# mcan1999/vulkan-raytracing

Measured on AMD Instinct MI355X. Metric: Mrays/sec (primary+secondary) at 1920×1080 depth 4; 1/2/4/8-GPU scaling, higher is better.
Workload: dtype f32

## Files before the change

### vulkan_raytracing_amd/csrc/kernels.hip

```cpp
#include <hip/hip_runtime.h>

#include "rt_kernels.h"
#include "../../include/rt_api.h"

namespace rt {

struct F3 { float x, y, z; };
__device__ __forceinline__ F3 mk3(float x, float y, float z) { F3 r; r.x = x; r.y = y; r.z = z; return r; }
__device__ __forceinline__ F3 add3(F3 a, F3 b) { return mk3(a.x + b.x, a.y + b.y, a.z + b.z); }
__device__ __forceinline__ F3 sub3(F3 a, F3 b) { return mk3(a.x - b.x, a.y - b.y, a.z - b.z); }
__device__ __forceinline__ F3 mul3(F3 a, float s) { return mk3(a.x * s, a.y * s, a.z * s); }
__device__ __forceinline__ F3 neg3(F3 a) { return mk3(-a.x, -a.y, -a.z); }
__device__ __forceinline__ float dot3(F3 a, F3 b) { return __builtin_fmaf(a.z, b.z, __builtin_fmaf(a.y, b.y, a.x * b.x)); }
__device__ __forceinline__ F3 cross3(F3 a, F3 b) {
  return mk3(__builtin_fmaf(a.y, b.z, -(a.z * b.y)), __builtin_fmaf(a.z, b.x, -(a.x * b.z)), __builtin_fmaf(a.x, b.y, -(a.y * b.x)));
}
__device__ __forceinline__ float length3(F3 v) { return __builtin_sqrtf(dot3(v, v)); }
__device__ __forceinline__ F3 normalize3(F3 v) { float inv = 1.0f / length3(v); return mul3(v, inv); }
__device__ __forceinline__ F3 fma3(float s, F3 a, F3 b) { return mk3(__builtin_fmaf(s, a.x, b.x), __builtin_fmaf(s, a.y, b.y), __builtin_fmaf(s, a.z, b.z)); }
__device__ __forceinline__ F3 reflect3(F3 I, F3 N) { float k = 2.0f * dot3(N, I); return fma3(-k, N, I); }

__device__ __forceinline__ F3 xform_point(const float* m, F3 p) {
  return mk3(__builtin_fmaf(m[2], p.z, __builtin_fmaf(m[1], p.y, m[0] * p.x)) + m[3],
             __builtin_fmaf(m[6], p.z, __builtin_fmaf(m[5], p.y, m[4] * p.x)) + m[7],
// ... 1159 lines not shown
    };
#else
    auto fast_step = [&]() {
      if (cur >= 0) {
        const uint4* np = reinterpret_cast<const uint4*>(node_bytes + ((uint32_t)cur << 5));
        const uint4 Q0 = np[0], Q1 = np[1];
        const int top = stk_lds[(sp - 1) * 64];
        const int2 ch = make_int2((int)Q1.z, (int)Q1.w);
        if (COUNT) cnt_nodes++;
        float t0, t1;
        const bool h0 = slab_q(Q0.x, Q0.y, Q0.z, qs, qb, rot, (RAYS8 ? tmin_ray : a.tmin), best_t, t0);
        const bool h1 = slab_q(Q0.w, Q1.x, Q1.y, qs, qb, rot, (RAYS8 ? tmin_ray : a.tmin), best_t, t1);
        const bool both = h0 && h1, none = !(h0 || h1), swap = t1 < t0;
        const uint32_t pm = 0u - (uint32_t)both;
        stk_lds[(((uint32_t)sp & pm) | ((uint32_t)STACK2_LDS & ~pm)) * 64u] = swap ? ch.x : ch.y;
        const int one = h0 ? ch.x : ch.y;
        cur = both ? (swap ? ch.y : ch.x) : (none ? top : one);
        sp += (both ? 1 : 0) - (none ? 1 : 0);
      }
    };
#endif
    constexpr int UNROLL = WIDE ? RT_WIDE_UNROLL : RT_INTERIOR_UNROLL;
    for (;;) {
      const uint32_t n_int = (uint32_t)__builtin_popcountll(__ballot(cur >= 0));
      if (n_int == 0 || n_int < keep_going) break;
#if !defined(RT_EXP_PHASE_SEL) && !defined(RT_EXP_VISIT_STAMPS)
      if (COUNT && lane == 0) { diag_iters++; diag_busy += n_int; }
#endif
      const bool deep = cur >= 0 && (sp + UNROLL > STACK2_LDS || far);
      if (!WIDE && __ballot(deep) == 0) {
#pragma unroll
        for (int r = 0; r < UNROLL; r++) fast_step();
      } else {
#pragma unroll
        for (int r = 0; r < UNROLL; r++) interior_step();
      }
    }

    PH_BEGIN(1)
    if (cur < 0 && cur > REF_MARK && cur_inst >= 0) {
      const bool any_ray = ANY || (QF && (qword & QF_TERMINATE) != 0u);
      for (int chain = 0; chain < RT_LEAF_CHAIN; chain++) {
        const uint32_t ref = (uint32_t)(~cur);
        const uint32_t first = ref >> 3, count = (ref & 7u) + 1u;
        for (uint32_t k = 0; k < count; k++) {
          const float4* tp = a.sc.tris + (size_t)(first + k) * 3;
          const float4 T0 = tp[0], T1 = tp[1], T2 = tp[2];
          if (COUNT) cnt_tris++;
          float tt, uu, vv;
          bool acc;
          if constexpr (QF) acc = tri_test_facing(T0, T1, T2, co, cd, tmin_ray, any_ray ? best_t : tmax, qword, tt, uu, vv);
          else acc = tri_test(T0, T1, T2, co, cd, (RAYS8 ? tmin_ray : a.tmin), (ANY ? best_t : ((ENTRY && MODE == MODE_CLOSEST) ? 10000.0f : tmax)), tt, uu, vv);
          if (acc) {
            if (ANY && MODE == MODE_SHADOW) best_inst = cur_inst;
            else {
              const int prim = (int)__float_as_uint(T2.y);
              const bool better = (best_inst < 0) || (tt < best_t) ||
                                  (tt == best_t && (cur_inst < best_inst || (cur_inst == best_inst && prim < best_prim)));
              if (better) { best_t = tt; best_u = uu; best_v = vv; best_prim = prim; best_inst = cur_inst; }
            }
          }
        }
        if (any_ray && best_inst >= 0) { cur = REF_DONE; break; }
        pop();
        if (!(cur < 0 && cur > REF_MARK)) break;
      }
    }
    PH_END(1)
    PH_BEGIN(2)
    if (cur == REF_MARK) {
      cur_inst = -1;
      pop();
      if (cur >= 0) { quant_space(wo, wd, a.sc.tlas_q_lo, a.sc.tlas_q_scale, qs, qb, rot); far = FAR && quant_far_o(wo, a.sc.tlas_q_lo, a.sc.tlas_q_scale); }
    }
    PH_END(2)
    PH_BEGIN(3)
    if (cur < 0 && cur > REF_MARK && cur_inst < 0) {
      const int ii = ~cur;
      int root; uint32_t imask;
      to_instance(ii, root, imask);
      bool skip = (imask & 0xFFu) == 0u;
      if (QF) {
        uint32_t cull;
        skip = !query_enters(qword, imask, cull);
        qword = (qword & ~(QF_CULL_NEG | QF_CULL_POS)) | cull;
      }
      if (skip) {
        pop();
        if (cur >= 0) { quant_space(wo, wd, a.sc.tlas_q_lo, a.sc.tlas_q_scale, qs, qb, rot); far = FAR && quant_far_o(wo, a.sc.tlas_q_lo, a.sc.tlas_q_scale); }
      } else {
        push(REF_MARK);
        cur_inst = ii; cur = root;
      }
    }

    PH_END(3)
    PH_BEGIN(4)
    const bool fin = !need && cur == REF_DONE;
    const uint64_t fin_mask = __ballot(fin);
    if (fin_mask != 0) {
      const uint32_t n_fin = (uint32_t)__builtin_popcountll(fin_mask);
      if (out_count + n_fin > 64u) flush();
      if (fin) {
        const uint32_t slot = out_count + prefix_rank(fin_mask);
        if (MODE == MODE_SHADOW) {
          s_out[wave][slot].x = best_inst < 0 ? 1.0f : 0.0f;
          s_outq[wave][slot] = make_int2((int)sid, (int)q);
        } else {
          s_out[wave][slot] = make_float4(best_t, best_u, best_v, __uint_as_float((uint32_t)best_prim));
          s_outq[wave][slot] = make_int2((int)q, best_inst);
        }
        need = true;
      }
      out_count += n_fin;
    }
    PH_END(4)
  }
  if (COUNT) {
    for (int off = 32; off > 0; off >>= 1) {
      cnt_nodes += __shfl_down((unsigned long long)cnt_nodes, off);
      cnt_tris += __shfl_down((unsigned long long)cnt_tris, off);
    }
    if (lane == 0) {
      const int off = ANY ? (CNT_NODE_VISITS_SH - CNT_NODE_VISITS) : 0;
      atomicAdd(reinterpret_cast<unsigned long long*>(a.counters + CNT_NODE_VISITS + off), (unsigned long long)cnt_nodes);
      atomicAdd(reinterpret_cast<unsigned long long*>(a.counters + CNT_TRI_TESTS + off), (unsigned long long)cnt_tris);
      const int dg = ANY ? CNT_DIAG_SH : CNT_DIAG;
      atomicAdd(reinterpret_cast<unsigned long long*>(a.counters + dg), (unsigned long long)diag_iters);
      atomicAdd(reinterpret_cast<unsigned long long*>(a.counters + dg + 2), (unsigned long long)diag_busy);
      atomicAdd(reinterpret_cast<unsigned long long*>(a.counters + dg + 4), (unsigned long long)(__builtin_readcyclecounter() - diag_t0));
    }
  }
}

template <int MODE, bool ANY, bool WIDE, bool ENTRY = false, bool FAR = true, bool CONT = false>
__global__ __launch_bounds__(256) __attribute__((amdgpu_waves_per_eu(RT_WAVES_PER_EU, RT_WAVES_PER_EU))) void k_trace(TraceArgs a) { trace_body<MODE, ANY, false, WIDE, ENTRY, FAR, CONT>(a); }
template <int MODE, bool ANY, bool WIDE, bool ENTRY = false, bool FAR = true, bool CONT = false>
__global__ __launch_bounds__(256) void k_trace_count(TraceArgs a) { trace_body<MODE, ANY, true, WIDE, ENTRY, FAR, CONT>(a); }

#ifdef RT_ALT_KERNELS
#include "kernels_alt.inc"
#include "kernels_tile.inc"
#endif

struct ShadeArgs {
  SceneDev sc;
  FrameDev f;
  UniformsDev u;
  int bounce;
  BatchTab bt;
};

struct Surface { F3 P, N; };
__device__ __forceinline__ Surface hit_surface(const SceneDev& sc, const InstanceDev* I, uint32_t prim, float hu, float hv) {
  const uint32_t* ix = sc.idx + I->first_index + 3u * prim;
  const uint32_t ia = ix[0], ib = ix[1], ic = ix[2];
  const float* vb = sc.verts + I->first_float;
  const float bx = (1.0f - hu) - hv, by = hu, bz = hv;
  const float* pa = vb + 6u * ia; const float* pb = vb + 6u * ib; const float* pc = vb + 6u * ic;
  const F3 pos = fma3(bz, mk3(pc[0], pc[1], pc[2]), fma3(by, mk3(pb[0], pb[1], pb[2]), mul3(mk3(pa[0], pa[1], pa[2]), bx)));
  const F3 nrm = fma3(bz, mk3(pc[3], pc[4], pc[5]), fma3(by, mk3(pb[3], pb[4], pb[5]), mul3(mk3(pa[3], pa[4], pa[5]), bx)));
  Surface s;
  s.P = xform_point(I->o2w, pos);
  s.N = normalize3(xform_normal(I->w2o, nrm));
  return s;
}

template <bool PIN> __device__ __forceinline__ float4 ambient_default() {
  float r = 0.08f;
  if constexpr (PIN) asm volatile("" : "+v"(r));
  return make_float4(r, 0.24f, r, 1.0f);
}
template <bool TILE, bool BATCH, bool RUNS, bool REG, typename A>
__device__ __forceinline__ void shade_slot(const A& a, const int bounce, const uint32_t shard, const uint32_t q, const bool in_range, const int inst_r, const float4 h_r) {
  const auto& f = a.f;
  const auto& U = a.u;
  const int cur = bounce & 1, nxt = cur ^ 1;
  const uint32_t lane = threadIdx.x & 63u;
  bool push_next = false, push_shadow = false, settled = false;
  F3 no = mk3(0, 0, 0), nd = mk3(0, 0, 1);
  float sh_tmax = 0.f; F3 sh_c = mk3(0, 0, 0); float sh_w = 0.f;
  uint32_t sh_ent = ENTRY_FROM_ROOT;
  uint32_t sid = SID_DEAD;
  int inst = HIT_DEAD;
  if (in_range) { if constexpr (REG) inst = inst_r; else inst = ld_stream(&f.hit_inst[q]); }
  if (inst != HIT_DEAD) {
    const float4 rd = ld_stream(&f.ray_d[cur][q]);
    sid = __float_as_uint(rd.w);
    const F3 d = mk3(rd.x, rd.y, rd.z);
    if (inst < 0) {
      const F3 c = sample_sky(a.sc, mk3(d.x, d.y, -d.z));
      st_stream(&f.sample_color[sid], make_float4(c.x, c.y, c.z, 1.0f));
    } else {
      float4 h = h_r;
      if constexpr (!REG) h = ld_stream(&f.hit_a[q]);
      const InstanceDev* I = a.sc.inst + inst;
      const uint32_t prim = __float_as_uint(h.w);
      const Surface S = hit_surface(a.sc, I, prim, h.y, h.z);
      const F3 P = S.P;
      F3 N = S.N;
      const int objectIndex = I->custom_index;
      uint32_t type = I->type != TYPE_BY_OBJECT_INDEX ? I->type : (objectIndex == 0 ? U.center_object_type : U.orbiting_object_type);
      const MaterialDev* M = nullptr;
      uint32_t mat = MATERIAL_NONE;
      if (a.sc.n_materials != 0) {
        mat = a.sc.prim_material[I->first_index / 3u + prim];
        M = a.sc.materials + mat;
        if (M->type != TYPE_BY_INSTANCE) type = M->type;
      }
      const bool last = (uint32_t)bounce >= U.max_bounce_count;
      if (type == 0u) {
        if (dot3(d, N) >= 0.0f) {
          st_stream(&f.sample_color[sid], ambient_default<REG>());
        } else {
          no = fma3(0.01f, N, P);
          F3 light = mk3(U.light_position[0], U.light_position[1], U.light_position[2]);
          float Iv = U.light_intensity;
          uint32_t fi = 0;
          if constexpr (BATCH) { fi = frame_of(sid, a.sc.batch_samples); light = mk3(a.bt.light[fi][0], a.bt.light[fi][1], a.bt.light[fi][2]); Iv = a.bt.light[fi][3]; }
          const F3 toL = sub3(light, P);
          const float dist = length3(toL);
          const F3 L = mul3(toL, 1.0f / dist);
          const F3 Hh = normalize3(add3(L, neg3(d)));
          const float NdotL = dot3(N, L), NdotH = dot3(N, Hh);
          const float dl = fmaxf(0.0f, NdotL);
          const float sp = M ? pow_int(fmaxf(0.0f, NdotH), (uint32_t)M->ns) : pow100(fmaxf(0.0f, NdotH));
          const uint32_t i = sid / (uint32_t)(f.rows * f.width) - fi * U.samples_per_pixel;
          float w = 1.0f;
          for (uint32_t k = 0; k < i; k++) w = w * 0.9f;
          const F3 kd = M ? mk3(M->kd[0], M->kd[1], M->kd[2]) : mk3(0.2f, 1.0f, 0.2f);
          const F3 ks = M ? mk3(M->ks[0], M->ks[1], M->ks[2]) : mk3(0.8f, 0.8f, 0.8f);
          const F3 diff = mk3((Iv * kd.x) * dl, (Iv * kd.y) * dl, (Iv * kd.z) * dl);
          const F3 spec = mk3((Iv * ks.x) * sp, (Iv * ks.y) * sp, (Iv * ks.z) * sp);
          const F3 amb = ambient_of(a.sc, mat);
          sh_c = fma3(w, add3(diff, spec), amb); sh_w = __uint_as_float(mat);
          nd = L; sh_tmax = dist;
          push_shadow = true;
          if (f.settle_dead_shadow_rays && __float_as_uint(sh_c.x) == __float_as_uint(amb.x) && __float_as_uint(sh_c.y) == __float_as_uint(amb.y) &&
              __float_as_uint(sh_c.z) == __float_as_uint(amb.z)) {
            st_stream(&f.sample_color[sid], make_float4(amb.x, amb.y, amb.z, 1.0f));
            push_shadow = false; settled = true;
          }
          if (f.light_entry != nullptr) {
            const F3 v = sub3(no, light);
            const float ax = __builtin_fabsf(v.x), ay = __builtin_fabsf(v.y), az = __builtin_fabsf(v.z);
            const int axis = (ax >= ay && ax >= az) ? 0 : (ay >= az ? 1 : 2);
            const float vc = axis == 0 ? v.x : (axis == 1 ? v.y : v.z), va = axis == 0 ? v.y : (axis == 1 ? v.z : v.x), vb = axis == 0 ? v.z : (axis == 1 ? v.x : v.y);
            const float c = __builtin_fabsf(vc);
            if (c > 0.0f) {
              const float T8 = (float)(8 * f.light_tiles);
              const float px = (va / c + 1.0f) * 0.5f * T8, py = (1.0f - vb / c) * 0.5f * T8;
              const int tx = min(max((int)(px * 0.125f), 0), f.light_tiles - 1), ty = min(max((int)(py * 0.125f), 0), f.light_tiles - 1);
              const int face = 2 * axis + (vc < 0.0f ? 1 : 0);
              sh_ent = (uint32_t)((face * f.light_tiles + ty) * f.light_tiles + tx) | (NdotL < 0.0f ? ENTRY_REVERSE : 0u);
            }
          }
        }
      } else if (type == 1u) {
        no = fma3(0.01f, N, P);
        nd = reflect3(d, N);
        push_next = true;
      } else if (type == 2u) {
        float ndoti = dot3(d, N);
        const bool outwards = ndoti > 0.0f;
        if (outwards) { N = neg3(N); ndoti = -ndoti; }
        const float ratio = M ? (outwards ? M->ni : 1.0f / M->ni) : (outwards ? 1.52f : (1.0f / 1.52f));
        const float k = 1.0f - (ratio * ratio) * (1.0f - ndoti * ndoti);
        if (k < 0.0f) { nd = reflect3(d, N); no = fma3(0.01f, N, P); }
        else {
          const float c = __builtin_fmaf(ratio, ndoti, __builtin_sqrtf(k));
          nd = normalize3(fma3(-c, N, mul3(d, ratio)));
          no = fma3(-0.01f, N, P);
        }
        push_next = true;
      } else {
        if (bounce == 0 && f.pixel_runs) {
          no = mk3(U.position[0], U.position[1], U.position[2]);
          if constexpr (BATCH) { const uint32_t fk = frame_of(sid, a.sc.batch_samples); no = mk3(a.bt.position[fk][0], a.bt.position[fk][1], a.bt.position[fk][2]); }
        } else {
          const float4 ro = ld_stream(&f.ray_o[cur][q]);
          no = mk3(ro.x, ro.y, ro.z);
        }
        nd = d; push_next = true;
      }
      if (push_next && last) {
        push_next = false;
        st_stream(&f.sample_color[sid], ambient_default<REG>());
      }
    }
  }
  {
    const uint64_t m_st = __ballot(settled);
    if (lane == 0 && m_st != 0ull) {
      __hip_atomic_fetch_add(f.counters + cnt_tail(Q_SHADOW0, (int)shard), (uint32_t)__builtin_popcountll(m_st), __ATOMIC_RELAXED, __HIP_MEMORY_SCOPE_AGENT);
      __hip_atomic_fetch_add(f.counters + cnt_work(Q_DEAD, (int)shard), (uint32_t)__builtin_popcountll(m_st), __ATOMIC_RELAXED, __HIP_MEMORY_SCOPE_AGENT);
    }
  }
  const uint32_t slot_n = wave_alloc(push_next, f.counters + cnt_tail(bounce + 1, (int)shard));
  if (push_next) {
    const uint32_t v = shard * f.shard_cap + slot_n;
    st_stream(&f.ray_o[nxt][v], make_float4(no.x, no.y, no.z, 10000.0f));
    st_stream(&f.ray_d[nxt][v], make_float4(nd.x, nd.y, nd.z, __uint_as_float(sid)));
  }
  if constexpr (RUNS) {
    if (in_range) {
      if (push_shadow) {
        st_stream(&f.sh_o[q], make_float4(no.x, no.y, no.z, sh_tmax));
        st_stream(&f.sh_c[q], make_float4(sh_c.x, sh_c.y, sh_c.z, sh_w));
        if (f.sh_e != nullptr) f.sh_e[q] = sh_ent;
      }
      st_stream(&f.sh_d[q], push_shadow ? make_float4(nd.x, nd.y, nd.z, __uint_as_float(sid)) : make_float4(0.f, 0.f, 0.f, __uint_as_float(SID_DEAD)));
    }
    const uint64_t m_sh = __ballot(push_shadow);
    if (lane == 0 && m_sh != 0ull) __hip_atomic_fetch_add(f.counters + cnt_tail(Q_SHADOW0, (int)shard), (uint32_t)__builtin_popcountll(m_sh), __ATOMIC_RELAXED, __HIP_MEMORY_SCOPE_AGENT);
  } else {
    const uint32_t slot_s = wave_alloc(push_shadow, f.counters + cnt_tail(Q_SHADOW, (int)shard));
    if (push_shadow) {
      const uint32_t v = f.sh_base + shard * f.shard_cap + slot_s;
      st_stream(&f.sh_o[v], make_float4(no.x, no.y, no.z, sh_tmax));
      st_stream(&f.sh_d[v], make_float4(nd.x, nd.y, nd.z, __uint_as_float(sid)));
      st_stream(&f.sh_c[v], make_float4(sh_c.x, sh_c.y, sh_c.z, sh_w));
      if (f.sh_e != nullptr) f.sh_e[v] = sh_ent;
    }
  }
}

template <bool TILE = false, bool BATCH = false, bool RUNS = false>
__device__ __forceinline__ void shade_body(const ShadeArgs& a, const int bounce) {
  const FrameDev& f = a.f;
  const UniformsDev& U = a.u;
  const uint32_t lane = threadIdx.x & 63u, wave = threadIdx.x >> 6;
  const int n_pass = TILE ? 2 : 1;
  for (int pass = 0; pass < n_pass; pass++) {
  uint32_t cnt[N_SHARDS], maxb = 0;
#pragma unroll
  for (int t = 0; t < N_SHARDS; t++) {
    if (TILE && pass) {
      uint32_t blobs = 0;
#pragma unroll
      for (int k = 0; k < BLOB_CLASSES; k++) blobs += ld_cursor(f.counters + cnt_tail(Q_BLOB_LIST + k, t));
      cnt[t] = blobs * (256u * ((U.samples_per_pixel + 3u) / 4u));
    } else cnt[t] = ld_cursor(f.counters + cnt_tail(bounce, t));
    maxb = max(maxb, (cnt[t] + 63u) >> 6);
  }
  const uint32_t n_waves = gridDim.x * 4u;
  for (uint32_t g = blockIdx.x * 4u + wave; g < maxb * N_SHARDS; g += n_waves) {
    const uint32_t shard = g & (N_SHARDS - 1), base = (g >> 3) << 6;
    uint32_t n = 0;
#pragma unroll
    for (int t = 0; t < N_SHARDS; t++) n = (shard == (uint32_t)t) ? cnt[t] : n;
    if (base >= n) continue;
    const uint32_t q = shard * f.shard_cap + ((TILE && pass) ? f.shard_cap - n : 0u) + base + lane;
    shade_slot<TILE, BATCH, RUNS, false>(a, bounce, shard, q, base + lane < n, HIT_DEAD, make_float4(0.f, 0.f, 0.f, 0.f));
  }
  }
}

template <bool TILE, bool BATCH, bool RUNS = false>
__global__ __launch_bounds__(256) void k_shade(ShadeArgs a) { shade_body<TILE, BATCH, RUNS>(a, a.bounce); }
// ... 583 lines not shown
```

### vulkan_raytracing_amd/csrc/kernels_beam.inc

```
struct BeamSpace { F3 s0, b0, s1, b1; uint3 rot; };

__device__ __forceinline__ bool slab_beam(uint32_t wx, uint32_t wy, uint32_t wz, const BeamSpace& B, float tmin, float tlim, float& tn) {
  wx = __builtin_amdgcn_alignbit(wx, wx, B.rot.x); wy = __builtin_amdgcn_alignbit(wy, wy, B.rot.y); wz = __builtin_amdgcn_alignbit(wz, wz, B.rot.z);
  const float nx = (float)(wx & 0xFFFFu), fx = (float)(wx >> 16), ny = (float)(wy & 0xFFFFu), fy = (float)(wy >> 16), nz = (float)(wz & 0xFFFFu), fz = (float)(wz >> 16);
  const float x0 = fminf(__builtin_fmaf(nx, B.s0.x, B.b0.x), __builtin_fmaf(nx, B.s1.x, B.b1.x)), x1 = fmaxf(__builtin_fmaf(fx, B.s0.x, B.b0.x), __builtin_fmaf(fx, B.s1.x, B.b1.x));
  const float y0 = fminf(__builtin_fmaf(ny, B.s0.y, B.b0.y), __builtin_fmaf(ny, B.s1.y, B.b1.y)), y1 = fmaxf(__builtin_fmaf(fy, B.s0.y, B.b0.y), __builtin_fmaf(fy, B.s1.y, B.b1.y));
  const float z0 = fminf(__builtin_fmaf(nz, B.s0.z, B.b0.z), __builtin_fmaf(nz, B.s1.z, B.b1.z)), z1 = fmaxf(__builtin_fmaf(fz, B.s0.z, B.b0.z), __builtin_fmaf(fz, B.s1.z, B.b1.z));
  tn = fmaxf(fmaxf(x0, y0), fmaxf(z0, tmin));
  const float tf = fminf(fminf(x1, y1), fminf(z1, tlim));
  return tn <= tf * 1.00002f;
}
__device__ __forceinline__ void beam_axis(float lo, float hi, float da, float t_far, float q_lo_minus_o, float q_scale, float& s0, float& b0, float& s1, float& b1, uint32_t& rot) {
  if (lo < 0.0f && hi > 0.0f) {
    const float K = 1.0e30f, inv = 1.0f / q_scale, r = t_far * da;
    const float U = (r - q_lo_minus_o) * inv + 1.0f, L = (-r - q_lo_minus_o) * inv - 1.0f;
    s0 = K; s1 = K; b0 = -K * U; b1 = -K * L; rot = 0u;
  }
  else { s0 = q_scale * lo; b0 = q_lo_minus_o * lo; s1 = q_scale * hi; b1 = q_lo_minus_o * hi; rot = lo < 0.0f ? 16u : 0u; }
}

#define RT_BEAM_EACH(M) M(0) M(1) M(2) M(3)
#ifndef RT_BEAM_KEEP_NUM
#define RT_BEAM_KEEP_NUM RT_KEEP_NUM
#endif
#ifndef RT_BEAM_UNROLL
#define RT_BEAM_UNROLL RT_INTERIOR_UNROLL
#endif

struct BeamShadeUniforms {
  float position[3], light_position[3], light_intensity;
  uint32_t max_bounce_count, samples_per_pixel, center_object_type, orbiting_object_type;
};
struct BeamShadeArgs {
  SceneDev sc;
  const float4* ray_o;
  const float4* ray_d;
  const uint32_t* tails;
  uint32_t* work;
  uint32_t shard_cap;
  int32_t* ovf_stack;
  uint32_t* counters;
  float tmin;
  const EntryRec* entry;
  float4* next_o;
  float4* next_d;
  float4* sh_o;
  float4* sh_d;
  float4* sh_c;
  uint32_t* sh_e;
  float4* sample_color;
  const EntryRec* light_entry;
  int width, rows, light_tiles, settle_dead_shadow_rays;
  BeamShadeUniforms u;
};
struct BeamShadeFrame {
  float4* ray_o[2]; float4* ray_d[2];
  float4* sh_o; float4* sh_d; float4* sh_c; uint32_t* sh_e;
  float4* sample_color;
  uint32_t* counters;
  const EntryRec* light_entry;
  uint32_t shard_cap;
  int width, rows, light_tiles, settle_dead_shadow_rays;
  static constexpr int pixel_runs = 64;
  static constexpr uint32_t sh_base = 0u;
};
struct BeamShadeView { const SceneDev& sc; const BeamShadeFrame& f; const BeamShadeUniforms& u; };

template <bool COUNT, bool SHADE = false, typename Args = TraceArgs>
__device__ __forceinline__ void beam_body(const Args& a, const uint32_t run) {
  __shared__ int s_stack[4][STACK2_LDS + 1][64];
  __shared__ float s_best[4][16][64];
  __shared__ float4 s_inst[LDS_INSTANCES ? LDS_INSTANCES : 1][5];
  const int n_lds_inst = a.sc.n_inst < LDS_INSTANCES ? a.sc.n_inst : LDS_INSTANCES;
  if ((int)threadIdx.x < n_lds_inst) {
    const InstanceDev* I = a.sc.inst + threadIdx.x;
    const float4* mp = reinterpret_cast<const float4*>(I->w2o);
    s_inst[threadIdx.x][0] = mp[0]; s_inst[threadIdx.x][1] = mp[1]; s_inst[threadIdx.x][2] = mp[2];
    s_inst[threadIdx.x][3] = make_float4(I->q_lo[0], I->q_lo[1], I->q_lo[2], __int_as_float(I->blas_root));
    s_inst[threadIdx.x][4] = make_float4(I->q_scale[0], I->q_scale[1], I->q_scale[2], __uint_as_float(I->mask));
  }
  __syncthreads();
  const uint32_t lane = threadIdx.x & 63u, wave = threadIdx.x >> 6;
  int* const stk = &s_stack[wave][0][lane];
  float* const bst = &s_best[wave][0][lane];
  const char* const node_bytes = reinterpret_cast<const char*>(a.sc.blas_nodes);
  const uint32_t S = run >> 6;
  uint64_t cnt_nodes = 0, cnt_tris = 0, diag_iters = 0, diag_busy = 0;
  const uint64_t diag_t0 = COUNT ? __builtin_readcyclecounter() : 0;
  uint32_t shard = blockIdx.x & (N_SHARDS - 1), tried = 0;

  for (;;) {
    uint32_t base = 0; bool got = false;
    while (tried < (uint32_t)N_SHARDS) {
      const uint32_t size = ld_cursor(a.tails + shard * CNT_STRIDE);
      uint32_t off = 0;
      if (lane == 0 && size) off = atomicAdd(a.work + shard * CNT_STRIDE, run);
      off = (uint32_t)__builtin_amdgcn_readfirstlane((int)off);
      if (size && off < size) { base = shard * a.shard_cap + off; got = true; break; }
      shard = (shard + 1u) & (N_SHARDS - 1); tried++;
    }
    if (!got) break;
    const uint32_t v0 = base + lane;

    uint32_t alive = 0, sid = 0;
    F3 co = mk3(0, 0, 0), cd0 = mk3(0, 0, 1), cd1 = cd0, cd2 = cd0, cd3 = cd0;
    float bt0 = -1.0f, bt1 = -1.0f, bt2 = -1.0f, bt3 = -1.0f;
    BeamSpace B;
    B.s0 = B.s1 = B.b0 = B.b1 = mk3(0, 0, 0); B.rot = make_uint3(0u, 0u, 0u);
    int cur = REF_DONE, sp = 1, cur_inst = -1;
    uint32_t my_visits = 0;

    auto push = [&](int v) {
      if (sp < STACK2_LDS) stk[sp * 64] = v;
      else *reinterpret_cast<volatile int32_t*>(a.ovf_stack + (size_t)(blockIdx.x * 256u + threadIdx.x) * a.sc.ovf_stride + (sp - STACK2_LDS)) = v;
      sp++;
    };
    auto pop = [&]() {
      sp--;
      if (sp < STACK2_LDS) cur = stk[sp * 64];
      else cur = *reinterpret_cast<volatile int32_t*>(a.ovf_stack + (size_t)(blockIdx.x * 256u + threadIdx.x) * a.sc.ovf_stride + (sp - STACK2_LDS));
    };
    auto set_space = [&](int ii, int& root, uint32_t& imask) {
      const float4 ro = a.ray_o[base];
      const F3 wo = mk3(ro.x, ro.y, ro.z);
      F3 w0 = mk3(0, 0, 1), w1 = w0, w2 = w0, w3 = w0;
#define RT_BEAM_LD(j) if (alive & (1u << j)) { const float4 r = a.ray_d[v0 + 64u * j]; w##j = mk3(r.x, r.y, r.z); }
      RT_BEAM_EACH(RT_BEAM_LD)
#undef RT_BEAM_LD
      float qlo3[3] = {a.sc.tlas_q_lo[0], a.sc.tlas_q_lo[1], a.sc.tlas_q_lo[2]}, qsc3[3] = {a.sc.tlas_q_scale[0], a.sc.tlas_q_scale[1], a.sc.tlas_q_scale[2]};
      root = 0; imask = 0xFFu;
      if (ii >= 0) {
        float4 m0, m1, m2, ql, qsc;
        if (ii < n_lds_inst) { m0 = s_inst[ii][0]; m1 = s_inst[ii][1]; m2 = s_inst[ii][2]; ql = s_inst[ii][3]; qsc = s_inst[ii][4]; }
        else {
          const InstanceDev* I = a.sc.inst + ii;
          const float4* mp = reinterpret_cast<const float4*>(I->w2o);
          m0 = mp[0]; m1 = mp[1]; m2 = mp[2];
          ql = make_float4(I->q_lo[0], I->q_lo[1], I->q_lo[2], __int_as_float(I->blas_root));
          qsc = make_float4(I->q_scale[0], I->q_scale[1], I->q_scale[2], __uint_as_float(I->mask));
        }
        root = __float_as_int(ql.w); imask = __float_as_uint(qsc.w);
        if ((imask & 0xFFu) == 0u) return;
        float m[12];
        m[0] = m0.x; m[1] = m0.y; m[2] = m0.z; m[3] = m0.w; m[4] = m1.x; m[5] = m1.y; m[6] = m1.z; m[7] = m1.w;
        m[8] = m2.x; m[9] = m2.y; m[10] = m2.z; m[11] = m2.w;
        co = xform_point(m, wo);
        cd0 = xform_vec(m, w0); cd1 = xform_vec(m, w1); cd2 = xform_vec(m, w2); cd3 = xform_vec(m, w3);
        qlo3[0] = ql.x; qlo3[1] = ql.y; qlo3[2] = ql.z; qsc3[0] = qsc.x; qsc3[1] = qsc.y; qsc3[2] = qsc.z;
      } else { co = wo; cd0 = w0; cd1 = w1; cd2 = w2; cd3 = w3; }
      float lx = 3.0e38f, ly = 3.0e38f, lz = 3.0e38f, hx = -3.0e38f, hy = -3.0e38f, hz = -3.0e38f, ax = 0.0f, ay = 0.0f, az = 0.0f, l2 = 3.0e38f;
#define RT_BEAM_ID(j) if (alive & (1u << j)) { const float ix = safe_rcp(cd##j.x), iy = safe_rcp(cd##j.y), iz = safe_rcp(cd##j.z); \
        lx = fminf(lx, ix); hx = fmaxf(hx, ix); ly = fminf(ly, iy); hy = fmaxf(hy, iy); lz = fminf(lz, iz); hz = fmaxf(hz, iz); \
        ax = fmaxf(ax, __builtin_fabsf(cd##j.x)); ay = fmaxf(ay, __builtin_fabsf(cd##j.y)); az = fmaxf(az, __builtin_fabsf(cd##j.z)); l2 = fminf(l2, dot3(cd##j, cd##j)); }
      RT_BEAM_EACH(RT_BEAM_ID)
#undef RT_BEAM_ID
      const float ex = fmaxf(__builtin_fabsf(qlo3[0] - co.x), __builtin_fabsf(__builtin_fmaf(65535.0f, qsc3[0], qlo3[0]) - co.x));
      const float ey = fmaxf(__builtin_fabsf(qlo3[1] - co.y), __builtin_fabsf(__builtin_fmaf(65535.0f, qsc3[1], qlo3[1]) - co.y));
      const float ez = fmaxf(__builtin_fabsf(qlo3[2] - co.z), __builtin_fabsf(__builtin_fmaf(65535.0f, qsc3[2], qlo3[2]) - co.z));
      const float t_far = fminf(10000.0f, 1.001f * __builtin_sqrtf((ex * ex + ey * ey + ez * ez) / fmaxf(l2, 1.0e-30f)));
      beam_axis(lx, hx, ax, t_far, qlo3[0] - co.x, qsc3[0], B.s0.x, B.b0.x, B.s1.x, B.b1.x, B.rot.x);
      beam_axis(ly, hy, ay, t_far, qlo3[1] - co.y, qsc3[1], B.s0.y, B.b0.y, B.s1.y, B.b1.y, B.rot.y);
      beam_axis(lz, hz, az, t_far, qlo3[2] - co.z, qsc3[2], B.s0.z, B.b0.z, B.s1.z, B.b1.z, B.rot.z);
    };

    {
#define RT_BEAM_ALIVE(j) if (j < S) { const float4 r = ld_stream(&a.ray_d[v0 + 64u * j]); if (r.x != 0.0f || r.y != 0.0f || r.z != 0.0f) { alive |= 1u << j; sid = __float_as_uint(r.w); } }
      RT_BEAM_EACH(RT_BEAM_ALIVE)
#undef RT_BEAM_ALIVE
    }
    if (alive & 1u) bt0 = 10000.0f;
    if (alive & 2u) bt1 = 10000.0f;
    if (alive & 4u) bt2 = 10000.0f;
    if (alive & 8u) bt3 = 10000.0f;
#pragma unroll
    for (int j = 0; j < 4; j++) { bst[(4 * j + 0) * 64] = 0.0f; bst[(4 * j + 1) * 64] = 0.0f; bst[(4 * j + 2) * 64] = __int_as_float(-1); bst[(4 * j + 3) * 64] = __int_as_float(-1); }
    stk[0] = REF_DONE;
    if (alive != 0u && a.entry == nullptr) {
      cur = a.sc.tlas_root + (a.sc.batch_samples ? (int)frame_of(sid, a.sc.batch_samples) * a.sc.tlas_stride : 0);
      int root; uint32_t imask;
      set_space(-1, root, imask);
    } else if (alive != 0u) {
      const uint32_t tile = __float_as_uint(ld_stream(&a.ray_o[base]).w);
      const int4* rp = reinterpret_cast<const int4*>(a.entry + tile);
      const int4 r0 = rp[0], r1 = rp[1];
      const uint32_t hdr = (uint32_t)r0.x;
      if (hdr != ENTRY_EMPTY) {
        const uint32_t nw = hdr & 15u, ia = hdr >> 8;
        const int wk[6] = {r0.z, r0.w, r1.x, r1.y, r1.z, r1.w};
#pragma unroll
        for (uint32_t k = 0; k < 6u; k++) if (k < nw) stk[(1u + k) * 64u] = wk[k];
        sp = 1 + (int)nw;
        cur = r0.y;
        int root; uint32_t imask;
        if (ia != ENTRY_NO_INST) { set_space((int)ia, root, imask); cur_inst = (int)ia; }
        else set_space(-1, root, imask);
      }
    }

    typedef __attribute__((address_space(3))) volatile int lds_vint;
    lds_vint* const stk_lds = (lds_vint*)stk;
    for (;;) {
      const uint32_t live = (uint32_t)__builtin_popcountll(__ballot(cur != REF_DONE));
      if (live == 0u) break;
      const uint32_t keep_going = (live * RT_BEAM_KEEP_NUM + 7u) >> 3;
      for (;;) {
        const uint32_t n_int = (uint32_t)__builtin_popcountll(__ballot(cur >= 0));
        if (n_int == 0u || n_int < keep_going) break;
        if (COUNT && lane == 0) { diag_iters++; diag_busy += n_int; }
        const float tlim = fmaxf(fmaxf(bt0, bt1), fmaxf(bt2, bt3));
        const bool deep = cur >= 0 && sp + RT_BEAM_UNROLL > STACK2_LDS;
        if (__ballot(deep) == 0ull) {
#pragma unroll
          for (int r = 0; r < RT_BEAM_UNROLL; r++)
            if (cur >= 0) {
              const uint4* np = reinterpret_cast<const uint4*>(node_bytes + ((uint32_t)cur << 5));
              const uint4 Q0 = np[0], Q1 = np[1];
              const int top = stk_lds[(sp - 1) * 64];
              const int2 ch = make_int2((int)Q1.z, (int)Q1.w);
              if (COUNT) { cnt_nodes++; my_visits++; }
              float t0, t1;
              const bool h0 = slab_beam(Q0.x, Q0.y, Q0.z, B, a.tmin, tlim, t0);
              const bool h1 = slab_beam(Q0.w, Q1.x, Q1.y, B, a.tmin, tlim, t1);
              const bool both = h0 && h1, none = !(h0 || h1), swap = t1 < t0;
              const uint32_t pm = 0u - (uint32_t)both;
              stk_lds[(((uint32_t)sp & pm) | ((uint32_t)STACK2_LDS & ~pm)) * 64u] = swap ? ch.x : ch.y;
              const int one = h0 ? ch.x : ch.y;
              cur = both ? (swap ? ch.y : ch.x) : (none ? top : one);
              sp += (both ? 1 : 0) - (none ? 1 : 0);
            }
        } else {
#pragma unroll
          for (int r = 0; r < RT_BEAM_UNROLL; r++)
            if (cur >= 0) {
              const uint4* np = reinterpret_cast<const uint4*>(node_bytes + ((uint32_t)cur << 5));
              const uint4 Q0 = np[0], Q1 = np[1];
              const int2 ch = make_int2((int)Q1.z, (int)Q1.w);
              if (COUNT) { cnt_nodes++; my_visits++; }
              float t0, t1;
              const bool h0 = slab_beam(Q0.x, Q0.y, Q0.z, B, a.tmin, tlim, t0);
              const bool h1 = slab_beam(Q0.w, Q1.x, Q1.y, B, a.tmin, tlim, t1);
              if (h0 && h1) { const bool swap = t1 < t0; push(swap ? ch.x : ch.y); cur = swap ? ch.y : ch.x; }
              else if (h0) cur = ch.x;
              else if (h1) cur = ch.y;
              else pop();
            }
        }
      }
      if (cur < 0 && cur > REF_MARK && cur_inst >= 0) {
        const uint32_t ref = (uint32_t)(~cur);
        const uint32_t first = ref >> 3, count = (ref & 7u) + 1u;
        for (uint32_t k = 0; k < count; k++) {
          const float4* tp = a.sc.tris + (size_t)(first + k) * 3;
          const float4 T0 = tp[0], T1 = tp[1], T2 = tp[2];
          const int prim = (int)__float_as_uint(T2.y);
#define RT_BEAM_TRI(j) if (alive & (1u << j)) { \
            if (COUNT) cnt_tris++; \
            float tt, uu, vv; \
            if (tri_test(T0, T1, T2, co, cd##j, a.tmin, 10000.0f, tt, uu, vv)) { \
              bool better = tt < bt##j; \
              if (tt == bt##j) { const int bi = __float_as_int(bst[(4 * j + 3) * 64]), bp = __float_as_int(bst[(4 * j + 2) * 64]); \
                                 better = bi < 0 || cur_inst < bi || (cur_inst == bi && prim < bp); } \
              if (better) { bt##j = tt; bst[(4 * j + 0) * 64] = uu; bst[(4 * j + 1) * 64] = vv; bst[(4 * j + 2) * 64] = __int_as_float(prim); bst[(4 * j + 3) * 64] = __int_as_float(cur_inst); } \
            } }
          RT_BEAM_EACH(RT_BEAM_TRI)
#undef RT_BEAM_TRI
        }
        pop();
      }
      if (cur == REF_MARK) {
        cur_inst = -1;
        pop();
        if (cur >= 0) { int root; uint32_t imask; set_space(-1, root, imask); }
      }
      if (cur < 0 && cur > REF_MARK && cur_inst < 0) {
        const int ii = ~cur;
        int root; uint32_t imask;
        set_space(ii, root, imask);
        if ((imask & 0xFFu) == 0u) {
          pop();
          if (cur >= 0) set_space(-1, root, imask);
        } else {
          push(REF_MARK);
          cur_inst = ii; cur = root;
        }
      }
    }

    if (COUNT) {
      uint32_t mx = my_visits;
      for (int off = 32; off > 0; off >>= 1) mx = max(mx, (uint32_t)__shfl_xor((int)mx, off));
      if (lane == 0) {
        atomicMax(a.counters + CNT_TILE_DIAG, mx);
        atomicAdd(reinterpret_cast<unsigned long long*>(a.counters + CNT_TILE_DIAG + 2), (unsigned long long)mx);
        atomicAdd(reinterpret_cast<unsigned long long*>(a.counters + CNT_TILE_DIAG + 4), 1ull);
      }
    }
    if constexpr (SHADE) {
      const uint32_t run_shard = (uint32_t)__builtin_amdgcn_readfirstlane((int)shard);
      const BeamShadeArgs* ka = (const BeamShadeArgs*)__builtin_amdgcn_kernarg_segment_ptr();
      asm volatile("" : "+s"(ka));
      const BeamShadeFrame sf{{const_cast<float4*>(ka->ray_o), ka->next_o}, {const_cast<float4*>(ka->ray_d), ka->next_d}, ka->sh_o, ka->sh_d, ka->sh_c, ka->sh_e, ka->sample_color,
                              ka->counters, ka->light_entry, ka->shard_cap, ka->width, ka->rows, ka->light_tiles, ka->settle_dead_shadow_rays};
      const BeamShadeView sv{ka->sc, sf, ka->u};
#pragma nounroll
      for (uint32_t j = 0; j < S; j++) {
        const float tj = j == 0u ? bt0 : (j == 1u ? bt1 : (j == 2u ? bt2 : bt3));
        const float* const b = bst + 256u * j;
        const int ij = (alive >> j) & 1u ? __float_as_int(b[192]) : HIT_DEAD;
        shade_slot<false, false, false, true>(sv, 0, run_shard, v0 + 64u * j, true, ij, make_float4(tj, b[0], b[64], b[128]));
      }
    } else {
#define RT_BEAM_OUT(j) if (j < S) { \
      const uint32_t v = v0 + 64u * j; \
      if (alive & (1u << j)) { \
        st_stream(&a.hit_a[v], make_float4(bt##j, bst[(4 * j + 0) * 64], bst[(4 * j + 1) * 64], bst[(4 * j + 2) * 64])); \
        st_stream(&a.hit_inst[v], __float_as_int(bst[(4 * j + 3) * 64])); \
      } else st_stream(&a.hit_inst[v], HIT_DEAD); }
    RT_BEAM_EACH(RT_BEAM_OUT)
#undef RT_BEAM_OUT
    }
  }
  if (COUNT) {
    for (int off = 32; off > 0; off >>= 1) {
      cnt_nodes += __shfl_down((unsigned long long)cnt_nodes, off);
      cnt_tris += __shfl_down((unsigned long long)cnt_tris, off);
    }
    if (lane == 0) {
      atomicAdd(reinterpret_cast<unsigned long long*>(a.counters + CNT_NODE_VISITS), (unsigned long long)cnt_nodes);
      atomicAdd(reinterpret_cast<unsigned long long*>(a.counters + CNT_TRI_TESTS), (unsigned long long)cnt_tris);
      atomicAdd(reinterpret_cast<unsigned long long*>(a.counters + CNT_DIAG), (unsigned long long)diag_iters);
      atomicAdd(reinterpret_cast<unsigned long long*>(a.counters + CNT_DIAG + 2), (unsigned long long)diag_busy);
      atomicAdd(reinterpret_cast<unsigned long long*>(a.counters + CNT_DIAG + 4), (unsigned long long)(__builtin_readcyclecounter() - diag_t0));
    }
  }
}

#ifndef RT_BEAM_WAVES
#define RT_BEAM_WAVES 4
#endif
__global__ __launch_bounds__(256) __attribute__((amdgpu_waves_per_eu(RT_BEAM_WAVES, RT_BEAM_WAVES))) void k_beam(TraceArgs a, uint32_t run) { beam_body<false>(a, run); }
__global__ __launch_bounds__(256) void k_beam_count(TraceArgs a, uint32_t run) { beam_body<true>(a, run); }
__global__ __launch_bounds__(256) __attribute__((amdgpu_waves_per_eu(RT_BEAM_WAVES, RT_BEAM_WAVES))) void k_beam_shade(BeamShadeArgs a, uint32_t run) { beam_body<false, true>(a, run); }

#ifdef RT_ALT_KERNELS
struct BeamShadowArgs {
  TraceArgs t;
  float light[3];
  uint32_t run;
};
struct BeamSpaceW { F3 s0, s1, n0, n1, f0, f1; uint3 rot; };

__device__ __forceinline__ bool slab_beam_w(uint32_t wx, uint32_t wy, uint32_t wz, const BeamSpaceW& B, float tmin, float tlim, float& tn, float& tfo) {
  wx = __builtin_amdgcn_alignbit(wx, wx, B.rot.x); wy = __builtin_amdgcn_alignbit(wy, wy, B.rot.y); wz = __builtin_amdgcn_alignbit(wz, wz, B.rot.z);
  const float nx = (float)(wx & 0xFFFFu), fx = (float)(wx >> 16), ny = (float)(wy & 0xFFFFu), fy = (float)(wy >> 16), nz = (float)(wz & 0xFFFFu), fz = (float)(wz >> 16);
  const float x0 = fminf(__builtin_fmaf(nx, B.s0.x, B.n0.x), __builtin_fmaf(nx, B.s1.x, B.n1.x)), x1 = fmaxf(__builtin_fmaf(fx, B.s0.x, B.f0.x), __builtin_fmaf(fx, B.s1.x, B.f1.x));
  const float y0 = fminf(__builtin_fmaf(ny, B.s0.y, B.n0.y), __builtin_fmaf(ny, B.s1.y, B.n1.y)), y1 = fmaxf(__builtin_fmaf(fy, B.s0.y, B.f0.y), __builtin_fmaf(fy, B.s1.y, B.f1.y));
  const float z0 = fminf(__builtin_fmaf(nz, B.s0.z, B.n0.z), __builtin_fmaf(nz, B.s1.z, B.n1.z)), z1 = fmaxf(__builtin_fmaf(fz, B.s0.z, B.f0.z), __builtin_fmaf(fz, B.s1.z, B.f1.z));
  tn = fmaxf(fmaxf(x0, y0), fmaxf(z0, tmin));
  const float tf = fminf(fminf(x1, y1), fminf(z1, tlim));
  tfo = tf;
  return tn <= tf * 1.00002f + 1.0e-6f;
}
__device__ __forceinline__ void beam_axis_w(float lo, float hi, float da, float t_far, float delta, float q_lo_minus_o, float q_scale,
                                            float& s0, float& s1, float& n0, float& n1, float& f0, float& f1, uint32_t& rot) {
  if (lo < 0.0f && hi > 0.0f) {
    const float K = 1.0e30f, inv = 1.0f / q_scale, r = __builtin_fmaf(t_far, da, delta);
    const float U = (r - q_lo_minus_o) * inv + 1.0f, L = (-r - q_lo_minus_o) * inv - 1.0f;
    s0 = K; s1 = K; n0 = -K * U; f0 = n0; n1 = -K * L; f1 = n1; rot = 0u;
  } else {
    s0 = q_scale * lo; s1 = q_scale * hi;
    const float b0 = q_lo_minus_o * lo, b1 = q_lo_minus_o * hi, e0 = delta * __builtin_fabsf(lo), e1 = delta * __builtin_fabsf(hi);
    n0 = b0 - e0; n1 = b1 - e1; f0 = b0 + e0; f1 = b1 + e1;
    rot = lo < 0.0f ? 16u : 0u;
  }
}

template <bool COUNT>
__device__ __forceinline__ void beam_shadow_body(const BeamShadowArgs& A) {
  const TraceArgs& a = A.t;
  __shared__ int s_stack[4][STACK2_LDS + 1][64];
  __shared__ float s_ray[4][24][64];
  __shared__ float4 s_inst[LDS_INSTANCES ? LDS_INSTANCES : 1][5];
  const int n_lds_inst = a.sc.n_inst < LDS_INSTANCES ? a.sc.n_inst : LDS_INSTANCES;
  if ((int)threadIdx.x < n_lds_inst) {
    const InstanceDev* I = a.sc.inst + threadIdx.x;
    const float4* mp = reinterpret_cast<const float4*>(I->w2o);
    s_inst[threadIdx.x][0] = mp[0]; s_inst[threadIdx.x][1] = mp[1]; s_inst[threadIdx.x][2] = mp[2];
    s_inst[threadIdx.x][3] = make_float4(I->q_lo[0], I->q_lo[1], I->q_lo[2], __int_as_float(I->blas_root));
    s_inst[threadIdx.x][4] = make_float4(I->q_scale[0], I->q_scale[1], I->q_scale[2], __uint_as_float(I->mask));
  }
  __syncthreads();
  const uint32_t lane = threadIdx.x & 63u, wave = threadIdx.x >> 6;
  int* const stk = &s_stack[wave][0][lane];
  float* const ray = &s_ray[wave][0][lane];
  const char* const node_bytes = reinterpret_cast<const char*>(a.sc.blas_nodes);
  const uint32_t S = A.run >> 6;
  uint64_t cnt_nodes = 0, cnt_tris = 0, diag_iters = 0, diag_busy = 0;
  const uint64_t diag_t0 = COUNT ? __builtin_readcyclecounter() : 0;
  uint32_t shard = blockIdx.x & (N_SHARDS - 1), tried = 0;

  for (;;) {
    uint32_t base = 0; bool got = false;
    while (tried < (uint32_t)N_SHARDS) {
      const uint32_t size = ld_cursor(a.tails + shard * CNT_STRIDE);
      uint32_t off = 0;
      if (lane == 0 && size) off = atomicAdd(a.work + shard * CNT_STRIDE, A.run);
      off = (uint32_t)__builtin_amdgcn_readfirstlane((int)off);
      if (size && off < size) { base = shard * a.shard_cap + off; got = true; break; }
      shard = (shard + 1u) & (N_SHARDS - 1); tried++;
    }
    if (!got) break;
    const uint32_t v0 = base + lane;
    uint32_t alive = 0, occluded = 0;
    float dt0 = -1.0f, dt1 = -1.0f, dt2 = -1.0f, dt3 = -1.0f;
#define RT_BEAM_ALIVE(j) if (j < S) { const float4 r = ld_stream(&a.ray_d[v0 + 64u * j]); if (r.x != 0.0f || r.y != 0.0f || r.z != 0.0f) { alive |= 1u << j; dt##j = ld_stream(&a.ray_o[v0 + 64u * j]).w; } }
    RT_BEAM_EACH(RT_BEAM_ALIVE)
#undef RT_BEAM_ALIVE
    uint32_t todo = alive, grp = 0;
    BeamSpaceW B;
    B.s0 = B.s1 = B.n0 = B.n1 = B.f0 = B.f1 = mk3(0, 0, 0); B.rot = make_uint3(0u, 0u, 0u);
    int cur = REF_DONE, sp = 1, cur_inst = -1;
    auto push = [&](int v) {
      if (sp < STACK2_LDS) stk[sp * 64] = v;
      else *reinterpret_cast<volatile int32_t*>(a.ovf_stack + (size_t)(blockIdx.x * 256u + threadIdx.x) * a.sc.ovf_stride + (sp - STACK2_LDS)) = v;
      sp++;
    };
    auto pop = [&]() {
      sp--;
      if (sp < STACK2_LDS) cur = stk[sp * 64];
      else cur = *reinterpret_cast<volatile int32_t*>(a.ovf_stack + (size_t)(blockIdx.x * 256u + threadIdx.x) * a.sc.ovf_stride + (sp - STACK2_LDS));
    };
    auto set_space = [&](int ii, int& root, uint32_t& imask) {
      float qlo3[3] = {a.sc.tlas_q_lo[0], a.sc.tlas_q_lo[1], a.sc.tlas_q_lo[2]}, qsc3[3] = {a.sc.tlas_q_scale[0], a.sc.tlas_q_scale[1], a.sc.tlas_q_scale[2]};
      float m[12] = {1.f, 0.f, 0.f, 0.f, 0.f, 1.f, 0.f, 0.f, 0.f, 0.f, 1.f, 0.f};
      root = 0; imask = 0xFFu;
      if (ii >= 0) {
        float4 m0, m1, m2, ql, qsc;
        if (ii < n_lds_inst) { m0 = s_inst[ii][0]; m1 = s_inst[ii][1]; m2 = s_inst[ii][2]; ql = s_inst[ii][3]; qsc = s_inst[ii][4]; }
        else {
          const InstanceDev* I = a.sc.inst + ii;
          const float4* mp = reinterpret_cast<const float4*>(I->w2o);
          m0 = mp[0]; m1 = mp[1]; m2 = mp[2];
          ql = make_float4(I->q_lo[0], I->q_lo[1], I->q_lo[2], __int_as_float(I->blas_root));
          qsc = make_float4(I->q_scale[0], I->q_scale[1], I->q_scale[2], __uint_as_float(I->mask));
        }
        root = __float_as_int(ql.w); imask = __float_as_uint(qsc.w);
        if ((imask & 0xFFu) == 0u) return;
        m[0] = m0.x; m[1] = m0.y; m[2] = m0.z; m[3] = m0.w; m[4] = m1.x; m[5] = m1.y; m[6] = m1.z; m[7] = m1.w;
        m[8] = m2.x; m[9] = m2.y; m[10] = m2.z; m[11] = m2.w;
        qlo3[0] = ql.x; qlo3[1] = ql.y; qlo3[2] = ql.z; qsc3[0] = qsc.x; qsc3[1] = qsc.y; qsc3[2] = qsc.z;
      }
      float lx = 3.0e38f, ly = 3.0e38f, lz = 3.0e38f, hx = -3.0e38f, hy = -3.0e38f, hz = -3.0e38f, ax = 0.0f, ay = 0.0f, az = 0.0f, l2 = 3.0e38f;
      float dmax = 0.0f;
      F3 E0 = mk3(0, 0, 0), E1 = E0, E2 = E0, E3 = E0;
#define RT_BEAM_RAY(j) if (grp & (1u << j)) { \
        const float4 o4 = a.ray_o[v0 + 64u * j], d4 = a.ray_d[v0 + 64u * j]; \
        const F3 wo = mk3(o4.x, o4.y, o4.z), wd = mk3(d4.x, d4.y, d4.z); \
        const F3 co = ii >= 0 ? xform_point(m, wo) : wo, cd = ii >= 0 ? xform_vec(m, wd) : wd; \
        ray[(6 * j + 0) * 64] = co.x; ray[(6 * j + 1) * 64] = co.y; ray[(6 * j + 2) * 64] = co.z; \
        ray[(6 * j + 3) * 64] = cd.x; ray[(6 * j + 4) * 64] = cd.y; ray[(6 * j + 5) * 64] = cd.z; \
        E##j = fma3(o4.w, cd, co);    \
        const float ix = safe_rcp(-cd.x), iy = safe_rcp(-cd.y), iz = safe_rcp(-cd.z); \
// ... 174 lines not shown
```

Baseline: 34950.

## Cache instance and vertex data across shade slots and reload kernargs via constant loads

Adds a per-lane ShadeCarry that keeps instance transforms and triangle vertex data in registers across the up-to-four shade slots of a beam run. When all lanes in the wave share one instance, that instance is preloaded with scalar constant loads. Kernel-argument pointers are now re-read through address-space-4 constant loads inside the run loop and through lazy pointer wrappers, so they do not stay live in registers. The aim is fewer redundant global loads during shading and lower register pressure, at the cost of carrying roughly 50 extra floats per lane, which could itself raise pressure.

```diff
diff --git a/vulkan_raytracing_amd/csrc/kernels.hip b/vulkan_raytracing_amd/csrc/kernels.hip
--- a/vulkan_raytracing_amd/csrc/kernels.hip
+++ b/vulkan_raytracing_amd/csrc/kernels.hip
@@ -1335,27 +1335,68 @@
 };
 
 struct Surface { F3 P, N; };
+__device__ __forceinline__ Surface surface_at(const float* o2w, const float* w2o, const float* pa, const float* pb, const float* pc, float hu, float hv) {
+  const float bx = (1.0f - hu) - hv, by = hu, bz = hv;
+  const F3 pos = fma3(bz, mk3(pc[0], pc[1], pc[2]), fma3(by, mk3(pb[0], pb[1], pb[2]), mul3(mk3(pa[0], pa[1], pa[2]), bx)));
+  const F3 nrm = fma3(bz, mk3(pc[3], pc[4], pc[5]), fma3(by, mk3(pb[3], pb[4], pb[5]), mul3(mk3(pa[3], pa[4], pa[5]), bx)));
+  Surface s;
+  s.P = xform_point(o2w, pos);
+  s.N = normalize3(xform_normal(w2o, nrm));
+  return s;
+}
 __device__ __forceinline__ Surface hit_surface(const SceneDev& sc, const InstanceDev* I, uint32_t prim, float hu, float hv) {
   const uint32_t* ix = sc.idx + I->first_index + 3u * prim;
   const uint32_t ia = ix[0], ib = ix[1], ic = ix[2];
   const float* vb = sc.verts + I->first_float;
-  const float bx = (1.0f - hu) - hv, by = hu, bz = hv;
-  const float* pa = vb + 6u * ia; const float* pb = vb + 6u * ib; const float* pc = vb + 6u * ic;
-  const F3 pos = fma3(bz, mk3(pc[0], pc[1], pc[2]), fma3(by, mk3(pb[0], pb[1], pb[2]), mul3(mk3(pa[0], pa[1], pa[2]), bx)));
-  const F3 nrm = fma3(bz, mk3(pc[3], pc[4], pc[5]), fma3(by, mk3(pb[3], pb[4], pb[5]), mul3(mk3(pa[3], pa[4], pa[5]), bx)));
-  Surface s;
-  s.P = xform_point(I->o2w, pos);
-  s.N = normalize3(xform_normal(I->w2o, nrm));
-  return s;
-}
+  return surface_at(I->o2w, I->w2o, vb + 6u * ia, vb + 6u * ib, vb + 6u * ic, hu, hv);
+}
+
+template <typename T> __device__ __forceinline__ T ld_const(const T* p) {
+  T v;
+  __builtin_memcpy(&v, (const __attribute__((address_space(4))) T*)p, sizeof(T));
+  return v;
+}
+template <typename T> __device__ __forceinline__ T* ld_const_ptr(T* const* p) {
+  typedef __attribute__((address_space(1))) T* global_ptr;
+  const __attribute__((address_space(4))) void* const c = (const __attribute__((address_space(4))) void*)(const void*)p;
+  return (T*)*static_cast<const __attribute__((address_space(4))) global_ptr*>(c);
+}
+
+struct InstanceShade { float w2o[12], o2w[12]; int32_t custom_index; uint32_t first_float, first_index, type; };
+struct ShadeCarry {
+  int inst = -1;
+  uint32_t prim = ~0u;
+  InstanceShade R = {};
+  float v[18] = {};
+  __device__ __forceinline__ void set_instance(int ii, const InstanceShade& r) { inst = ii; prim = ~0u; R = r; }
+  __device__ __forceinline__ static InstanceShade fields_of(const InstanceDev& I) {
+    InstanceShade r;
+#pragma unroll
+    for (int k = 0; k < 12; k++) { r.w2o[k] = I.w2o[k]; r.o2w[k] = I.o2w[k]; }
+    r.custom_index = I.custom_index; r.first_float = I.first_float; r.first_index = I.first_index; r.type = I.type;
+    return r;
+  }
+  __device__ __forceinline__ void fetch(const SceneDev& sc, int ii, uint32_t pp) {
+    if (ii != inst) set_instance(ii, fields_of(sc.inst[ii]));
+    if (pp != prim) {
+      const uint32_t* ix = sc.idx + R.first_index + 3u * pp;
+      const uint32_t ia = ix[0], ib = ix[1], ic = ix[2];
+      const float* vb = sc.verts + R.first_float;
+      const float* pa = vb + 6u * ia; const float* pb = vb + 6u * ib; const float* pc = vb + 6u * ic;
+#pragma unroll
+      for (int k = 0; k < 6; k++) { v[k] = pa[k]; v[6 + k] = pb[k]; v[12 + k] = pc[k]; }
+      prim = pp;
+    }
+  }
+};
 
 template <bool PIN> __device__ __forceinline__ float4 ambient_default() {
   float r = 0.08f;
   if constexpr (PIN) asm volatile("" : "+v"(r));
   return make_float4(r, 0.24f, r, 1.0f);
 }
-template <bool TILE, bool BATCH, bool RUNS, bool REG, typename A>
-__device__ __forceinline__ void shade_slot(const A& a, const int bounce, const uint32_t shard, const uint32_t q, const bool in_range, const int inst_r, const float4 h_r) {
+template <bool TILE, bool BATCH, bool RUNS, bool REG, typename A, typename RC = void>
+__device__ __forceinline__ void shade_slot(const A& a, const int bounce, const uint32_t shard, const uint32_t q, const bool in_range, const int inst_r, const float4 h_r, RC* carry = nullptr) {
   const auto& f = a.f;
   const auto& U = a.u;
   const int cur = bounce & 1, nxt = cur ^ 1;
@@ -1377,17 +1418,26 @@
     } else {
       float4 h = h_r;
       if constexpr (!REG) h = ld_stream(&f.hit_a[q]);
-      const InstanceDev* I = a.sc.inst + inst;
       const uint32_t prim = __float_as_uint(h.w);
-      const Surface S = hit_surface(a.sc, I, prim, h.y, h.z);
+      Surface S;
+      int objectIndex;
+      uint32_t inst_type, first_index;
+      if constexpr (REG) {
+        carry->fetch(a.sc, inst, prim);
+        S = surface_at(carry->R.o2w, carry->R.w2o, carry->v, carry->v + 6, carry->v + 12, h.y, h.z);
+        objectIndex = carry->R.custom_index; inst_type = carry->R.type; first_index = carry->R.first_index;
+      } else {
+        const InstanceDev* I = a.sc.inst + inst;
+        S = hit_surface(a.sc, I, prim, h.y, h.z);
+        objectIndex = I->custom_index; inst_type = I->type; first_index = I->first_index;
+      }
       const F3 P = S.P;
       F3 N = S.N;
-      const int objectIndex = I->custom_index;
-      uint32_t type = I->type != TYPE_BY_OBJECT_INDEX ? I->type : (objectIndex == 0 ? U.center_object_type : U.orbiting_object_type);
+      uint32_t type = inst_type != TYPE_BY_OBJECT_INDEX ? inst_type : (objectIndex == 0 ? U.center_object_type : U.orbiting_object_type);
       const MaterialDev* M = nullptr;
       uint32_t mat = MATERIAL_NONE;
       if (a.sc.n_materials != 0) {
-        mat = a.sc.prim_material[I->first_index / 3u + prim];
+        mat = a.sc.prim_material[first_index / 3u + prim];
         M = a.sc.materials + mat;
         if (M->type != TYPE_BY_INSTANCE) type = M->type;
       }
diff --git a/vulkan_raytracing_amd/csrc/kernels_beam.inc b/vulkan_raytracing_amd/csrc/kernels_beam.inc
--- a/vulkan_raytracing_amd/csrc/kernels_beam.inc
+++ b/vulkan_raytracing_amd/csrc/kernels_beam.inc
@@ -53,21 +53,39 @@
   int width, rows, light_tiles, settle_dead_shadow_rays;
   BeamShadeUniforms u;
 };
+template <typename T> struct KargPtr {
+  T* const* at;
+  T* held;
+  __device__ __forceinline__ operator T*() const { return at != nullptr ? ld_const_ptr(at) : held; }
+};
 struct BeamShadeFrame {
-  float4* ray_o[2]; float4* ray_d[2];
-  float4* sh_o; float4* sh_d; float4* sh_c; uint32_t* sh_e;
-  float4* sample_color;
-  uint32_t* counters;
-  const EntryRec* light_entry;
+  KargPtr<float4> ray_o[2], ray_d[2];
+  KargPtr<float4> sh_o, sh_d, sh_c; KargPtr<uint32_t> sh_e;
+  KargPtr<float4> sample_color;
+  KargPtr<uint32_t> counters;
+  KargPtr<const EntryRec> light_entry;
   uint32_t shard_cap;
   int width, rows, light_tiles, settle_dead_shadow_rays;
   static constexpr int pixel_runs = 64;
   static constexpr uint32_t sh_base = 0u;
 };
-struct BeamShadeView { const SceneDev& sc; const BeamShadeFrame& f; const BeamShadeUniforms& u; };
+struct BeamShadeScene {
+  const BeamShadeArgs* ka;
+  int n_materials;
+  KargPtr<const MaterialDev> materials;
+  KargPtr<const uint32_t> prim_material;
+  __device__ __forceinline__ operator SceneDev() const {
+    SceneDev s = ld_const(&ka->sc);
+    s.inst = ld_const_ptr(&ka->sc.inst); s.verts = ld_const_ptr(&ka->sc.verts); s.idx = ld_const_ptr(&ka->sc.idx); s.sky = ld_const_ptr(&ka->sc.sky);
+    s.materials = ld_const_ptr(&ka->sc.materials); s.prim_material = ld_const_ptr(&ka->sc.prim_material);
+    return s;
+  }
+};
+struct BeamShadeView { const BeamShadeScene& sc; const BeamShadeFrame& f; const BeamShadeUniforms& u; };
 
 template <bool COUNT, bool SHADE = false, typename Args = TraceArgs>
-__device__ __forceinline__ void beam_body(const Args& a, const uint32_t run) {
+__device__ __forceinline__ void beam_body(const Args& a_entry, const uint32_t run) {
+  const Args& a = a_entry;
   __shared__ int s_stack[4][STACK2_LDS + 1][64];
   __shared__ float s_best[4][16][64];
   __shared__ float4 s_inst[LDS_INSTANCES ? LDS_INSTANCES : 1][5];
@@ -83,13 +101,23 @@
   const uint32_t lane = threadIdx.x & 63u, wave = threadIdx.x >> 6;
   int* const stk = &s_stack[wave][0][lane];
   float* const bst = &s_best[wave][0][lane];
-  const char* const node_bytes = reinterpret_cast<const char*>(a.sc.blas_nodes);
   const uint32_t S = run >> 6;
   uint64_t cnt_nodes = 0, cnt_tris = 0, diag_iters = 0, diag_busy = 0;
   const uint64_t diag_t0 = COUNT ? __builtin_readcyclecounter() : 0;
   uint32_t shard = blockIdx.x & (N_SHARDS - 1), tried = 0;
 
   for (;;) {
+    Args a_run;
+    if constexpr (SHADE) {
+      const Args* ka = (const Args*)__builtin_amdgcn_kernarg_segment_ptr();
+      asm volatile("" : "+s"(ka));
+      a_run = ld_const(ka);
+      a_run.sc.blas_nodes = ld_const_ptr(&ka->sc.blas_nodes); a_run.sc.tris = ld_const_ptr(&ka->sc.tris); a_run.sc.inst = ld_const_ptr(&ka->sc.inst);
+      a_run.ray_o = ld_const_ptr(&ka->ray_o); a_run.ray_d = ld_const_ptr(&ka->ray_d); a_run.tails = ld_const_ptr(&ka->tails); a_run.work = ld_const_ptr(&ka->work);
+      a_run.ovf_stack = ld_const_ptr(&ka->ovf_stack); a_run.entry = ld_const_ptr(&ka->entry);
+    }
+    const Args& a = SHADE ? a_run : a_entry;
+    const char* const node_bytes = reinterpret_cast<const char*>(a.sc.blas_nodes);
     uint32_t base = 0; bool got = false;
     while (tried < (uint32_t)N_SHARDS) {
       const uint32_t size = ld_cursor(a.tails + shard * CNT_STRIDE);
@@ -299,15 +327,35 @@
       const uint32_t run_shard = (uint32_t)__builtin_amdgcn_readfirstlane((int)shard);
       const BeamShadeArgs* ka = (const BeamShadeArgs*)__builtin_amdgcn_kernarg_segment_ptr();
       asm volatile("" : "+s"(ka));
-      const BeamShadeFrame sf{{const_cast<float4*>(ka->ray_o), ka->next_o}, {const_cast<float4*>(ka->ray_d), ka->next_d}, ka->sh_o, ka->sh_d, ka->sh_c, ka->sh_e, ka->sample_color,
-                              ka->counters, ka->light_entry, ka->shard_cap, ka->width, ka->rows, ka->light_tiles, ka->settle_dead_shadow_rays};
-      const BeamShadeView sv{ka->sc, sf, ka->u};
+      ShadeCarry carry;
+      {
+        int first = -1; bool agree = true;
+#pragma unroll
+        for (uint32_t j = 0; j < 4u; j++) {
+          const int ij = (alive >> j) & 1u ? __float_as_int(bst[(4u * j + 3u) * 64u]) : -1;
+          if (ij >= 0) { agree = agree && (first < 0 || ij == first); if (first < 0) first = ij; }
+        }
+        const uint64_t m_hit = __ballot(first >= 0);
+        if (m_hit != 0ull) {
+          const int one = __builtin_amdgcn_readlane(first, (int)__builtin_ctzll(m_hit));
+          if (__ballot(first >= 0 && !(agree && first == one)) == 0ull) carry.set_instance(one, ShadeCarry::fields_of(ld_const(ld_const_ptr(&ka->sc.inst) + one)));
+        }
+      }
+      asm volatile("" : "+s"(ka));
+      const BeamShadeFrame sf{{{const_cast<float4* const*>(&ka->ray_o), nullptr}, {&ka->next_o, nullptr}},
+                              {{nullptr, const_cast<float4*>(ld_const_ptr(&ka->ray_d))}, {&ka->next_d, nullptr}},
+                              {&ka->sh_o, nullptr}, {&ka->sh_d, nullptr}, {&ka->sh_c, nullptr}, {&ka->sh_e, nullptr},
+                              {nullptr, ld_const_ptr(&ka->sample_color)}, {nullptr, ld_const_ptr(&ka->counters)}, {&ka->light_entry, nullptr},
+                              ld_const(&ka->shard_cap), ld_const(&ka->width), ld_const(&ka->rows), ld_const(&ka->light_tiles), ld_const(&ka->settle_dead_shadow_rays)};
+      const BeamShadeScene sg{ka, ld_const(&ka->sc.n_materials), {&ka->sc.materials, nullptr}, {&ka->sc.prim_material, nullptr}};
+      const BeamShadeUniforms su = ld_const(&ka->u);
+      const BeamShadeView sv{sg, sf, su};
 #pragma nounroll
       for (uint32_t j = 0; j < S; j++) {
         const float tj = j == 0u ? bt0 : (j == 1u ? bt1 : (j == 2u ? bt2 : bt3));
         const float* const b = bst + 256u * j;
         const int ij = (alive >> j) & 1u ? __float_as_int(b[192]) : HIT_DEAD;
-        shade_slot<false, false, false, true>(sv, 0, run_shard, v0 + 64u * j, true, ij, make_float4(tj, b[0], b[64], b[128]));
+        shade_slot<false, false, false, true>(sv, 0, run_shard, v0 + 64u * j, true, ij, make_float4(tj, b[0], b[64], b[128]), &carry);
       }
     } else {
 #define RT_BEAM_OUT(j) if (j < S) { \
```

After: 35770, median of 6. +2.4%, better.
